# KogarashiNetwork/dusk-plonk

Hardware: AMD Instinct MI355X
Metric: PLONK prover constraints/sec (BLS12-381) at n=2^16 and 2^20, 1/2/4/8 GPUs (higher is better)
Workload: dtype u32-limb Montgomery Fr/Fp (integer)

## Files before the change

### dusk-plonk_amd/csrc/debug.hip

```cpp
#include <hip/hip_runtime.h>

#include <algorithm>
#include <vector>

#include "g1r.hpp"
#include "internal.hpp"
#include "prover.hpp"

namespace plk {
namespace {

template <class C>
__global__ void k_field_op(int op, const Fe<C>* __restrict__ a, const Fe<C>* __restrict__ b,
                           Fe<C>* __restrict__ out, uint64_t n) {
  const uint64_t i = (uint64_t)blockIdx.x * blockDim.x + threadIdx.x;
  if (i >= n) return;
  const Fe<C> x = a[i], y = b[i];
  Fe<C> r;
  switch (op) {
    case 0: r = fe_mul(x, y); break;
    case 1: r = fe_add(x, y); break;
    case 2: r = fe_sub(x, y); break;
    case 3: r = fe_sqr(x); break;
    default: r = fe_inv(x); break;
// ... 531 lines not shown
    plk::DeviceGuard g(key->ctx->device);
    hipStream_t s = key->ctx->stream;
    plk::DevBuf din, dout;
    int st;
    if ((st = din.alloc(len * sizeof(plk::Fr))) || (st = dout.alloc(total * sizeof(plk::Fr))))
      return st;
    PLK_HIP_TRY(hipMemcpyAsync(din.ptr, coef, len * sizeof(plk::Fr), hipMemcpyHostToDevice, s));
    plk::NttBatch b;
    b.in_stride = 0;
    b.out_stride = n;
    b.pre = key->coset_s.as<plk::Fr>();
    b.pre_stride = n + 8;
    if ((st = plk::ntt_run_batch(key->dom, din.as<plk::Fr>(), dout.as<plk::Fr>(), len, 1, 1,
                                 nullptr, s, (uint32_t)key->qb, b)))
      return st;
    PLK_HIP_TRY(hipMemcpyAsync(out, dout.ptr, total * sizeof(plk::Fr), hipMemcpyDeviceToHost, s));
    PLK_HIP_TRY(plk::stream_wait(s));
    return PLK_OK;
  } catch (...) {
    return PLK_E_DEVICE;
  }
}

extern "C" int plk_debug_prover_stage(plk_ctx* ctx, int stage, const uint64_t* const* in,
                                      const size_t* in_len, size_t n_in, const plk_fr* scalars,
                                      size_t n_scalars, const uint64_t* params, size_t n_params,
                                      uint64_t* out, size_t out_cap) {
  try {
    if (!ctx || stage < 0 || stage >= plk::kStCount) return PLK_E_ARG;
    if ((n_in && (!in || !in_len)) || (n_scalars && !scalars) || (n_params && !params) ||
        (out_cap && !out) || n_in > 32)
      return PLK_E_ARG;
    for (size_t k = 0; k < n_in; ++k)
      if (in_len[k] > ((size_t)1 << 28) || (in_len[k] && !in[k])) return PLK_E_ARG;
    const plk::StageCall c{stage, in, in_len, n_in, scalars, n_scalars, params, n_params, out, out_cap};
    plk::DeviceGuard g(ctx->device);
    return plk::run_stage(ctx, c);
  } catch (...) {
    return PLK_E_DEVICE;
  }
}
```

### dusk-plonk_amd/csrc/prover.hip

```cpp
#include <hip/hip_runtime.h>

#include <algorithm>
#include <cstring>
#include <memory>
#include <mutex>
#include <vector>

#include "ffr.hpp"
#include "internal.hpp"
#include "msm_common.hpp"
#include "prover.hpp"
#include "transcript.hpp"

using namespace plk;

namespace {

Fr fr_u64(uint64_t v) {
  Fr x = fe_zero<FrCfg>();
  x.v[0] = (uint32_t)v;
  x.v[1] = (uint32_t)(v >> 32);
  return fe_to_mont(x);
}
Fr fr_from(const plk_fr& a) {
// ... 267 lines not shown
  const size_t max_points = std::min<size_t>(std::min<size_t>(key->srs->n, key->n_trim), cap);
  std::vector<size_t> use(lens.size());
  for (size_t i = 0; i < lens.size(); ++i) use[i] = std::min(lens[i], max_points);
  int overall = PLK_OK;
  for (size_t base = 0; base < ptrs.size(); base += kMaxSlots) {
    const size_t m = std::min<size_t>(kMaxSlots, ptrs.size() - base);
    const int r = msm_run_batch(key->srs, ws, ptrs.data() + base, use.data() + base,
                                lens.data() + base, m, outs + base,
                                statuses ? statuses + base : nullptr, s, 0, 1, 0,
                                info ? info + base : nullptr);
    if (r != PLK_OK && r != PLK_E_DEGREE) return r;
    if (r != PLK_OK) overall = r;
  }
  return overall;
}

uint32_t lagrange_bucket_max(const plk_srs* s, size_t len) {
  const size_t dense = (size_t)s->windows * len >> (s->c - 1);
  return (uint32_t)std::max<size_t>(4 * kChunkMax, 4 * dense);
}

bool lagrange_commit_enabled() {
  const char* e = getenv("PLK_LAGRANGE_COMMIT");
  return !(e && e[0] == '0' && e[1] == 0);
}

int shard_commit(plk_prover* P, const std::vector<const Fr*>& ptrs,
                 const std::vector<size_t>& lens, plk_g1* outs, int* statuses, size_t cap) {
  plk_key* key = P->key;
  const size_t cnt = ptrs.size();
  const size_t max_points = std::min<size_t>(std::min<size_t>(key->srs->n, key->n_trim), cap);
  const bool buckets = P->shard_buckets;
  plk_srs* srs = buckets ? key->srs : P->shard;
  const uint64_t lo = buckets ? 0 : P->shard_lo, hi = buckets ? key->srs->n : lo + P->shard->n;
  const bool last = buckets || P->rank == P->world - 1;
  const uint32_t part = buckets ? (uint32_t)P->rank : 0, parts = buckets ? (uint32_t)P->world : 1;
  std::vector<const Fr*> lp(cnt);
  std::vector<size_t> luse(cnt), lchk(cnt);
  int local = PLK_OK;
  if (last && hi < max_points) local = PLK_E_ARG;
  for (size_t i = 0; i < cnt; ++i) {
    const size_t use = std::min(lens[i], max_points);
    luse[i] = use > lo ? (size_t)(std::min<uint64_t>(use, hi) - lo) : 0;
    lchk[i] = luse[i];
    lp[i] = ptrs[i] + lo;
    if (last && lens[i] > use) {
// ... 101 lines not shown
  qa.vk = fe_sqr(ch.var_sep);
  qa.vk2 = fe_sqr(qa.vk);
  qa.edwards_d = edwards_d();
  qa.has_fixed = has_fixed ? 1 : 0;
  qa.has_var = has_var ? 1 : 0;
  for (int j = 0; j < blocks; ++j) qa.vh_inv[j] = vh_inv[j];
  auto em1 = [](const Fr& x) { return fe_to_rx_domain(x); };
  auto em2 = [](const Fr& x) { return fe_to_rx_domain(fe_to_rx_domain(x)); };
  const Fr one = fe_one<FrCfg>(), two = fe_dbl(one);
  for (int mb = 0; mb < blocks; ++mb) qa.rx_bg[mb] = em2(fe_mul(ch.beta, s_m[mb]));
  qa.rx_beta = em2(ch.beta);
  qa.rx_gamma = em1(ch.gamma);
  qa.rx_one_w = em1(one);
  qa.rx_two_w = em1(two);
  qa.rx_three_w = em1(fe_add(two, one));
  qa.rx_kappa = em1(qa.kappa);
  qa.rx_kappa2 = em1(qa.kappa2);
  qa.rx_kappa3 = em1(qa.kappa3);
  qa.rx_alpha2 = em1(alpha2);
  for (int j = 0; j < blocks; ++j) qa.rx_vh[j] = em2(vh_inv[j]);
  qa.rx_32 = fr_u64(32);
  qa.rx_inv32 = fe_inv(qa.rx_32);
}
}

namespace plk {
namespace {
__global__ void k_sigma_values(const uint32_t* __restrict__ codes, const Fr* __restrict__ el,
                               uint64_t n, Fr k1, Fr k2, Fr k3, Fr* __restrict__ out) {
  const uint64_t i = (uint64_t)blockIdx.x * blockDim.x + threadIdx.x;
  if (i >= 4 * n) return;
  const uint32_t code = codes[i];
  const uint32_t g = code >> 2, col = code & 3;
  Fr v = el[g];
  if (col == 1) v = fe_mul(v, k1);
  if (col == 2) v = fe_mul(v, k2);
  if (col == 3) v = fe_mul(v, k3);
  out[i] = v;
}
}
}

extern "C" {

namespace {
std::mutex g_pool_mu;
// ... 336 lines not shown
    {
      const Fr gq = key->dom->g, one = fe_one<FrCfg>();
      Fr w8n;
      fr_root_of_unity(k + 3, w8n);
      const uint64_t rowc = n + 8;
      TRY(key->coset_s.alloc(QB * rowc * sizeof(Fr)));
      TRY(key->coset_w.alloc(QB * rowc * sizeof(Fr)));
      TRY(key->coset_pi.alloc(QB * rowc * sizeof(Fr)));
      TRY(key->icoset_q.alloc(QB * n * sizeof(Fr)));
      const Fr c32 = fr_u64(32);
      Fr sm = gq;
      for (int mb = 0; mb < QB; ++mb) {
        key->s_m[mb] = sm;
        TRY(ntt_power_table(key->coset_s.as<Fr>() + mb * rowc, sm, one, rowc, true, s));
        TRY(ntt_power_table(key->coset_w.as<Fr>() + mb * rowc, sm, c32, rowc, true, s));
        TRY(ntt_power_table(key->coset_pi.as<Fr>() + mb * rowc, sm, fe_inv(c32), rowc, true, s));
        TRY(ntt_power_table(key->icoset_q.as<Fr>() + mb * n, fe_inv(sm), key->dom->n_inv, n, true,
                            s));
        sm = fe_mul(sm, w8n);
      }
      Fr cm[kQBlocksMax];
      for (int mb = 0; mb < QB; ++mb) {
        cm[mb] = fe_pow_u64(key->s_m[mb], n);
        key->vh_inv[mb] = fe_inv(fe_sub(cm[mb], one));
      }
      for (int mb = 0; mb < QB; ++mb) {
        Fr poly[kQBlocksMax + 1];
        int deg = 0;
        poly[0] = one;
        Fr den = one;
        for (int j = 0; j < QB; ++j) {
          if (j == mb) continue;
          poly[deg + 1] = fe_zero<FrCfg>();
          for (int l = deg + 1; l >= 1; --l)
            poly[l] = fe_sub(poly[l - 1], fe_mul(poly[l], cm[j]));
          poly[0] = fe_neg(fe_mul(poly[0], cm[j]));
          ++deg;
          den = fe_mul(den, fe_sub(cm[mb], cm[j]));
        }
        const Fr dinv = fe_inv(den);
        for (int l = 0; l < QB; ++l) key->comb.m[l * QB + mb] = fe_to_rx_domain(fe_mul(poly[l], dinv));
      }
    }
    auto coset_fwd = [&](const Fr* in, Fr* out, uint64_t len, const DevBuf& table) {
      NttBatch b;
      b.in_stride = 0;
      b.out_stride = n;
      b.pre = table.as<Fr>();
      b.pre_stride = n + 8;
      return ntt_run_batch(key->dom, in, out, len, 1, 1, nullptr, s, QB, b);
    };
    TRY(key->selq.alloc(SEL_COUNTQ * nq * sizeof(Fr)));
    const int sel_src[SEL_COUNTQ] = {QM, QL, QR, QO, Q4, QC, QARITH, QRANGE, QLOGIC, QFIXED, QVAR};
    const bool sel_used[SEL_COUNTQ] = {true, true, true, true, true, true, true, key->has_range,
                                       key->has_logic, key->has_fixed, key->has_var};
    for (int j = 0; j < SEL_COUNTQ; ++j)
      if (sel_used[j])
        TRY(coset_fwd(qc + sel_src[j] * n, key->selq.as<Fr>() + j * nq, n, key->coset_s));
    TRY(key->sigmaq.alloc(4 * nq * sizeof(Fr)));
    for (int c = 0; c < 4; ++c)
      TRY(coset_fwd(sc + c * n, key->sigmaq.as<Fr>() + c * nq, n, key->coset_s));
    TRY(key->l1q.alloc(nq * sizeof(Fr)));
    {
      DevBuf tmp;
      TRY(tmp.alloc(n * sizeof(Fr)));
      TRY(pk_fill(tmp.as<Fr>(), key->dom->n_inv, n, s));
      TRY(coset_fwd(tmp.as<Fr>(), key->l1q.as<Fr>(), n, key->coset_s));
      PLK_HIP_TRY(stream_wait(s));
    }
    std::vector<uint32_t> idx(4 * n, 0);
    for (uint64_t i = 0; i < m; ++i)
      for (int c = 0; c < 4; ++c) {
        idx[c * n + i] = cs->gates[i].w[c];
        key->max_wire = std::max(key->max_wire, cs->gates[i].w[c]);
      }
    key->struct_hash = cs->struct_hash;
    TRY(key->wire_idx.alloc(4 * n * 4));
    PLK_HIP_TRY(hipMemcpyAsync(key->wire_idx.ptr, idx.data(), 4 * n * 4, hipMemcpyHostToDevice, s));
    PLK_HIP_TRY(stream_wait(s));
    *out = key.release();
    return PLK_OK;
  } catch (const std::bad_alloc&) {
    return PLK_E_OOM;
  } catch (...) {
    return PLK_E_DEVICE;
  }
}

int plk_key_destroy(plk_key* key) {
  if (!key) return PLK_E_ARG;
  DeviceGuard g(key->ctx->device);
  (void)stream_wait(key->ctx->stream);
  delete key;
  return PLK_OK;
}

int plk_key_info(const plk_key* key, uint64_t* n, uint64_t* m, plk_g1* commitments) {
  if (!key) return PLK_E_ARG;
  if (n) *n = key->n;
  if (m) *m = key->m;
  if (commitments) std::memcpy(commitments, key->comms, sizeof key->comms);
  return PLK_OK;
}

int plk_prover_create(plk_key* key, plk_prover** out) {
  try {
    if (!key || !out) return PLK_E_ARG;
    *out = nullptr;
    DeviceGuard guard(key->ctx->device);
    std::unique_ptr<plk_prover> p(new plk_prover());
    p->key = key;
    p->ws = msm_workspace_new();
    if (!p->ws->tail_forced) p->ws->tail_quad = lane_tail_policy(key->n);
    p->ws->shared_chip = true;
    PLK_HIP_TRY(hipStreamCreateWithFlags(&p->stream, hipStreamNonBlocking));
    p->own_stream = true;
    *out = p.release();
    return PLK_OK;
  } catch (const std::bad_alloc&) {
    return PLK_E_OOM;
  }
}

int plk_prover_destroy(plk_prover* p) {
// ... 126 lines not shown
    for (uint64_t i = 0; i < m; ++i)
      if (cs->gates[i].code & kPiBit) pis.emplace_back(i, gate_unpack(cs, i).pi);
    for (auto& p : pis) tr.append_scalar("pi", p.second);
    if (pi_count) *pi_count = pis.size();
    if (public_inputs)
      for (size_t i = 0; i < pis.size() && i < pi_cap; ++i) public_inputs[i] = fr_to(pis[i].second);

    {
      const size_t bytes = cs->witness.size() * sizeof(Fr);
      TRY(P->pin_witness.alloc(bytes));
      const size_t chunk = 8u << 20;
      const char* src = reinterpret_cast<const char*>(cs->witness.data());
      char* pin = P->pin_witness.as<char>();
      char* dst = P->witness.as<char>();
      for (size_t off = 0; off < bytes; off += chunk) {
        const size_t len = std::min(chunk, bytes - off);
        std::memcpy(pin + off, src + off, len);
        PLK_HIP_TRY(hipMemcpyAsync(dst + off, pin + off, len, hipMemcpyHostToDevice, s));
      }
    }
    Fr* wl = P->wires_lag.as<Fr>();
    Fr* wc = P->wires_coef.as<Fr>();
    TRY(pk_gather_wires(P->witness.as<Fr>(), key->wire_idx.as<uint32_t>(), m, n, wl, S, s));
    {
      NttBatch b;
      b.in_stride = S;
      b.out_stride = S;
      TRY(ntt_run_batch(key->dom, wl, wc, n, -1, 0, nsc, s, 4, b));
    }
    BlindBatch bb{};
    bb.npoly = 4;
    for (int c = 0; c < 4; ++c) {
      bb.poly[c] = wc + c * S;
      bb.lag[c] = wl + c * S;
      bb.b[c].count = 2;
      bb.b[c].r[0] = rng.fr();
      bb.b[c].r[1] = rng.fr();
    }
    TRY(pk_blind_batch(bb, n, s));
    plk_g1 wcom[4];
    {
      bool coef[4] = {true, true, true, true};
      for (int c = 0; c < 4; ++c) P->commit_basis[c] = 0, P->commit_entries[c] = 0;
      if (key->lag && !P->shard && !P->shard_buckets) {
        const Fr* ptrs[4] = {wl, wl + S, wl + 2 * S, wl + 3 * S};
        const size_t lens[4] = {n + 2, n + 2, n + 2, n + 2};
        MsmSlotInfo info[4];
        TRY(msm_run_batch(key->lag, *P->ws, ptrs, lens, lens, 4, wcom, nullptr, s, 0, 1,
                          lagrange_bucket_max(key->lag, n + 2), info));
        for (int c = 0; c < 4; ++c) {
          coef[c] = info[c].hot;
// ... 64 lines not shown
        pd.c[i] = fe_mul(pis[i].second, key->dom->n_inv);
      }
      TRY(pk_pi_coef(pd, key->dom->tw_inv.as<Fr>(), n, P->pi_coef.as<Fr>(), s));
    } else if (!pis.empty() && !pi_sparse) {
      PLK_HIP_TRY(hipMemsetAsync(pil, 0, n * sizeof(Fr), s));
      for (size_t i = 0; i < pis.size(); ++i) {
        P->pin_small.as<Fr>()[i] = pis[i].second;
        PLK_HIP_TRY(hipMemcpyAsync(pil + pis[i].first, P->pin_small.as<Fr>() + i, sizeof(Fr),
                                   hipMemcpyHostToDevice, s));
      }
    }
    Fr* ev = P->evq.as<Fr>();
    auto coset_fwd = [&](const Fr* in, Fr* out, uint64_t len, const DevBuf& table) {
      NttBatch b;
      b.in_stride = 0;
      b.out_stride = n;
      b.pre = table.as<Fr>();
      b.pre_stride = n + 8;
      return ntt_run_batch(key->dom, in, out, len, 1, 1, nsc, s, QB, b);
    };
    if (!pis.empty() && !pi_direct && !pi_sparse)
      TRY(ntt_run(key->dom, pil, P->pi_coef.as<Fr>(), n, -1, 0, nsc, s, 1));
    TRY(coset_fwd(zc, ev + 0 * nq, n + 3, key->coset_s));
    {
      NttBatch b;
      b.group = QB;
      b.in_stride = 0;
      b.in_group_stride = S;
      b.out_stride = n;
      b.pre = key->coset_w.as<Fr>();
      b.pre_stride = n + 8;
      TRY(ntt_run_batch(key->dom, wc, ev + nq, n + 2, 1, 1, nsc, s, 4 * QB, b));
    }
    if (pi_sparse) {
      PiSparse ps{};
      ps.count = (uint32_t)pis.size();
      for (size_t i = 0; i < pis.size(); ++i) {
        ps.idx[i] = (uint32_t)pis[i].first;
        ps.v[i] = pis[i].second;
      }
      TRY(pk_pi_sparse(ps, key->l1q.as<Fr>(), key->k, nq, ev + 5 * nq, s));
    } else if (!pis.empty()) {
      TRY(coset_fwd(P->pi_coef.as<Fr>(), ev + 5 * nq, n, key->coset_pi));
    }
    const Fr alpha2 = fe_sqr(alpha);
    QuotientArgs qa{};
    qa.z = ev;
    qa.a = ev + nq;
    qa.b = ev + 2 * nq;
    qa.c = ev + 3 * nq;
    qa.d = ev + 4 * nq;
    qa.pi = pis.empty() ? nullptr : ev + 5 * nq;
    qa.l1 = key->l1q.as<Fr>();
    qa.sel = key->selq.as<Fr>();
    qa.sigma = key->sigmaq.as<Fr>();
    qa.elements = key->dom->tw_fwd.as<Fr>();
// ... 252 lines not shown
```

### dusk-plonk_amd/csrc/prover.hpp

```cpp
#pragma once
#include <map>
#include <string>
#include <vector>

#include "internal.hpp"

namespace plk {

struct BlindArgs {
  Fr r[4];
  uint32_t count;
};
constexpr int kPiDirect = 16;
struct PiDirect {
  uint64_t idx[kPiDirect];
  Fr c[kPiDirect];
  uint32_t count;
};
struct BlindBatch {
  Fr* poly[4];
  Fr* lag[4];
  BlindArgs b[4];
  uint32_t npoly;
};

enum { SEL_QM = 0, SEL_QL, SEL_QR, SEL_QO, SEL_Q4, SEL_QC, SEL_QARITH, SEL_QRANGE, SEL_QLOGIC,
       SEL_QFIXED, SEL_QVAR, SEL_COUNTQ };

constexpr int kQBlocks = 5, kQBlocksSmall = 6, kQBlocksMax = 6;
inline int q_blocks(uint64_t n) { return n >= 16 ? kQBlocks : kQBlocksSmall; }
constexpr int kPiSparse = 4;
struct PiSparse {
  uint32_t count;
  uint32_t idx[kPiSparse];
  Fr v[kPiSparse];
};

struct QuotientArgs {
  const Fr *a, *b, *c, *d, *z, *pi, *l1, *sel, *sigma, *elements;
  Fr* out;
  uint64_t nq;
  uint32_t log_blk;
  Fr g, alpha, alpha2, beta, gamma, k1, k2, k3;
  Fr range_sep, kappa, kappa2, kappa3;
  Fr logic_sep, lk, lk2, lk3, lk4;
  Fr fixed_sep, fk, fk2, fk3;
  Fr var_sep, vk, vk2;
  Fr edwards_d;
  int has_range, has_logic, has_fixed, has_var;
  Fr vh_inv[kQBlocksMax];
  Fr rx_bg[kQBlocksMax], rx_beta, rx_gamma;
  Fr rx_one_w, rx_two_w, rx_three_w;
  Fr rx_kappa, rx_kappa2, rx_kappa3;
// ... 65 lines not shown
  return id;
}

PLK_HD Fr widget_var_base(const Fr& x1, const Fr& x3, const Fr& y1, const Fr& y3, const Fr& x2,
                          const Fr& y2, const Fr& x1y2, const Fr& k, const Fr& k2, const Fr& d) {
  const Fr xy_consistency = fe_sub(fe_mul(x1, y2), x1y2);
  const Fr y1x2 = fe_mul(y1, x2);
  const Fr y1y2 = fe_mul(y1, y2);
  const Fr x1x2 = fe_mul(x1, x2);
  const Fr dprod = fe_mul(fe_mul(d, x1y2), y1x2);
  const Fr x3c = fe_sub(fe_add(x1y2, y1x2), fe_add(x3, fe_mul(x3, dprod)));
  const Fr y3c = fe_sub(fe_add(y1y2, x1x2), fe_sub(y3, fe_mul(y3, dprod)));
  return fe_add(fe_add(xy_consistency, fe_mul(x3c, k)), fe_mul(y3c, k2));
}

int pk_gather_wires(const Fr* witness, const uint32_t* idx, uint64_t m, uint64_t n, Fr* out,
                    uint64_t stride, hipStream_t s);
int pk_blind(Fr* poly, uint64_t n, const BlindArgs& b, hipStream_t s);
int pk_blind_batch(const BlindBatch& bb, uint64_t n, hipStream_t s);
int pk_pi_coef(const PiDirect& pd, const Fr* tw_inv, uint64_t n, Fr* out, hipStream_t s);
int pk_pi_sparse(const PiSparse& ps, const Fr* l1, uint32_t log_n, uint64_t nq, Fr* out,
                 hipStream_t s);
int pk_fill(Fr* out, const Fr& v, uint64_t n, hipStream_t s);
int pk_perm_numden(const Fr* wires, uint64_t wire_stride, const Fr* sigmas, const Fr* elements,
                   uint64_t n, const Fr& beta, const Fr& gamma, const Fr& k1, const Fr& k2, const Fr& k3,
                   Fr* num, Fr* den, hipStream_t s);
int pk_mul3(const Fr* a, const Fr* b, const Fr& c, Fr* out, uint64_t n, hipStream_t s);
uint64_t pk_scan_tmp_elems(uint64_t n);
int pk_scan(const Fr* in, Fr* out, uint64_t n, bool mul, bool suffix, bool exclusive, Fr* tmp,
            hipStream_t s);
int pk_quotient(const QuotientArgs& q, hipStream_t s);
struct CombineMat {
  Fr m[kQBlocksMax * kQBlocksMax];
};
int pk_coset_combine(const Fr* in, uint64_t n, int blocks, const CombineMat& mat, Fr* out,
                     hipStream_t s);
int pk_scale_copy(const Fr* in, const Fr& c, Fr* out, uint64_t n, hipStream_t s);
uint32_t pk_eval_max_blocks(uint64_t max_len);
int pk_eval(const EvalBatch& e, uint32_t count, uint64_t max_len, Fr* partial, Fr* d_out,
            hipStream_t s);
int pk_lincomb(const LinComb& lc, Fr* out, uint64_t len_out, hipStream_t s);
int pk_scale_powers(const Fr* c, uint64_t len, const Fr& x, uint64_t shift, Fr* y, hipStream_t s);
int pk_ruffini(const Fr* c, uint64_t len, const Fr& z, Fr* q, Fr* tmp, Fr* scan_tmp,
               hipStream_t s);

struct Gate {
// ... 26 lines not shown

struct plk_key {
  plk_ctx* ctx = nullptr;
  plk_srs* srs = nullptr;
  std::string label;
  uint64_t m = 0, n = 0, n_trim = 0;
  uint32_t k = 0;
  plk_domain* dom = nullptr;
  plk_srs* lag = nullptr;
  int qb = 0;
  bool has_range = false, has_logic = false, has_fixed = false, has_var = false;
  plk::DevBuf q_coef;
  plk::DevBuf selq;
  plk::DevBuf sigma_coef;
  plk::DevBuf sigma_lag;
  plk::DevBuf sigmaq;
  plk::DevBuf l1q;
  plk::DevBuf coset_s, coset_w, coset_pi;
  plk::DevBuf icoset_q;
  plk::Fr s_m[plk::kQBlocksMax];
  plk::CombineMat comb;
  plk::DevBuf wire_idx;
  plk::Fr vh_inv[plk::kQBlocksMax];
  plk_g1 comms[15];
  uint64_t struct_hash = 0;
  uint32_t max_wire = 0;
  std::mutex def_mu;
  std::unique_ptr<plk_prover> def_prover;
  ~plk_key();
};

struct plk_prover {
  plk_key* key = nullptr;
  hipStream_t stream = nullptr;
  bool own_stream = false;
  plk::MsmWorkspace* ws = nullptr;
  plk_srs* shard = nullptr;
  uint64_t shard_lo = 0;
  bool shard_buckets = false;
  int rank = 0, world = 1;
  plk_allgather_fn allgather = nullptr;
  void* allgather_user = nullptr;
  plk::PinnedBuf pin_witness, pin_small;
  plk::PinnedBuf eval_out;
  void* eval_dev = nullptr;
  int commit_basis[4] = {0, 0, 0, 0};
// ... 6 lines not shown
```

### dusk-plonk_amd/csrc/prover_kernels.hip

```cpp
#include <hip/hip_runtime.h>

#include "ffr.hpp"
#include "internal.hpp"
#include "prover.hpp"

namespace plk {

namespace {

__device__ __forceinline__ Fr ldf(const Fr* p) {
  const uint4* q = reinterpret_cast<const uint4*>(p);
  uint4 a = q[0], b = q[1];
  Fr r;
  r.v[0] = a.x; r.v[1] = a.y; r.v[2] = a.z; r.v[3] = a.w;
  r.v[4] = b.x; r.v[5] = b.y; r.v[6] = b.z; r.v[7] = b.w;
  return r;
}

__device__ __forceinline__ void stf(Fr* p, const Fr& v) {
  uint4* q = reinterpret_cast<uint4*>(p);
  q[0] = make_uint4(v.v[0], v.v[1], v.v[2], v.v[3]);
  q[1] = make_uint4(v.v[4], v.v[5], v.v[6], v.v[7]);
}

// ... 46 lines not shown
    acc = rx_add(acc, rx_mul(rx_unpack(pd.c[k]), ldr(&tw_inv[(pd.idx[k] * j) & (n - 1)])));
  stf(&out[j], rx_pack_canonical(acc));
}

__global__ void __launch_bounds__(256) k_pi_sparse(PiSparse ps, const Fr* __restrict__ l1,
                                                   uint32_t log_n, uint64_t nq,
                                                   Fr* __restrict__ out) {
  const uint64_t i = (uint64_t)blockIdx.x * blockDim.x + threadIdx.x;
  if (i >= nq) return;
  const uint64_t mask = (1ull << log_n) - 1, base = i & ~mask, u = i & mask;
  RFr acc = rx_mul(ldr(&l1[base + ((u - ps.idx[0]) & mask)]), rx_unpack(ps.v[0]));
  for (uint32_t k = 1; k < ps.count; ++k)
    acc = rx_add(acc, rx_mul(ldr(&l1[base + ((u - ps.idx[k]) & mask)]), rx_unpack(ps.v[k])));
  stf(&out[i], rx_pack_canonical(acc));
}

__global__ void k_blind_batch(BlindBatch bb, uint64_t n) {
  const uint32_t p = threadIdx.x >> 2, i = threadIdx.x & 3;
  if (p >= bb.npoly || i >= bb.b[p].count) return;
  Fr* poly = bb.poly[p];
  stf(&poly[i], fe_sub(ldf(&poly[i]), bb.b[p].r[i]));
  stf(&poly[n + i], bb.b[p].r[i]);
  if (bb.lag[p]) stf(&bb.lag[p][n + i], bb.b[p].r[i]);
}

__global__ void k_fill(Fr* __restrict__ out, Fr v, uint64_t n) {
  const uint64_t i = (uint64_t)blockIdx.x * blockDim.x + threadIdx.x;
  if (i < n) stf(&out[i], v);
}

__global__ void k_perm_numden(const Fr* __restrict__ wires, uint64_t ws, const Fr* __restrict__ sigmas,
                              const Fr* __restrict__ elements, uint64_t n, Fr beta_rx, Fr gamma,
                              Fr k1_rx, Fr k2_rx, Fr k3_rx, Fr fix, Fr* __restrict__ num,
                              Fr* __restrict__ den) {
  const uint64_t i = (uint64_t)blockIdx.x * blockDim.x + threadIdx.x;
  if (i >= n) return;
  const RFr be = rx_unpack(beta_rx), g = rx_unpack(gamma);
  const RFr bx = rx_mul(be, ldr(&elements[i]));
  auto tn = [&](int c, const RFr& bxk) { return add3_u(ldr(&wires[c * ws + i]), g, bxk); };
  auto td = [&](int c) { return add3_u(ldr(&wires[c * ws + i]), g, rx_mul(be, ldr(&sigmas[c * n + i]))); };
  RFr nu = rx_norm(tn(0, bx)), de = rx_norm(td(0));
  nu = rx_mul(nu, tn(1, rx_mul(rx_unpack(k1_rx), bx)));
  de = rx_mul(de, td(1));
  nu = rx_mul(nu, tn(2, rx_mul(rx_unpack(k2_rx), bx)));
  de = rx_mul(de, td(2));
  nu = rx_mul(nu, tn(3, rx_mul(rx_unpack(k3_rx), bx)));
// ... 486 lines not shown

int pk_pi_coef(const PiDirect& pd, const Fr* tw_inv, uint64_t n, Fr* out, hipStream_t s) {
  if (pd.count > (uint32_t)kPiDirect || (n & (n - 1))) return PLK_E_ARG;
  hipLaunchKernelGGL(k_pi_coef, dim3(blocks_for(n, 256)), dim3(256), 0, s, pd, tw_inv, n, out);
  PLK_HIP_TRY(hipGetLastError());
  return PLK_OK;
}

int pk_pi_sparse(const PiSparse& ps, const Fr* l1, uint32_t log_n, uint64_t nq, Fr* out,
                 hipStream_t s) {
  if (ps.count == 0 || ps.count > (uint32_t)kPiSparse) return PLK_E_ARG;
  hipLaunchKernelGGL(k_pi_sparse, dim3(blocks_for(nq, 256)), dim3(256), 0, s, ps, l1, log_n, nq,
                     out);
  PLK_HIP_TRY(hipGetLastError());
  return PLK_OK;
}

int pk_blind_batch(const BlindBatch& bb, uint64_t n, hipStream_t s) {
  hipLaunchKernelGGL(k_blind_batch, dim3(1), dim3(64), 0, s, bb, n);
  PLK_HIP_TRY(hipGetLastError());
  return PLK_OK;
}

int pk_fill(Fr* out, const Fr& v, uint64_t n, hipStream_t s) {
  hipLaunchKernelGGL(k_fill, dim3(blocks_for(n, 256)), dim3(256), 0, s, out, v, n);
  PLK_HIP_TRY(hipGetLastError());
  return PLK_OK;
}

int pk_perm_numden(const Fr* wires, uint64_t wire_stride, const Fr* sigmas, const Fr* elements,
                   uint64_t n, const Fr& beta, const Fr& gamma, const Fr& k1, const Fr& k2, const Fr& k3,
                   Fr* num, Fr* den, hipStream_t s) {
  Fr fix = fe_zero<FrCfg>();
  fix.v[0] = 1;
  for (int b = 0; b < 4 * RxShape<FrCfg>::B * RxShape<FrCfg>::L - 3 * 256; ++b) fix = fe_dbl(fix);
  hipLaunchKernelGGL(k_perm_numden, dim3(blocks_for(n, 256)), dim3(256), 0, s, wires, wire_stride,
                     sigmas, elements, n, fe_to_rx_domain(beta), gamma, fe_to_rx_domain(k1),
                     fe_to_rx_domain(k2), fe_to_rx_domain(k3), fix, num, den);
  PLK_HIP_TRY(hipGetLastError());
  return PLK_OK;
}

int pk_mul3(const Fr* a, const Fr* b, const Fr& c, Fr* out, uint64_t n, hipStream_t s) {
  hipLaunchKernelGGL(k_mul3, dim3(blocks_for(n, 256)), dim3(256), 0, s, a, b, c, out, n);
  PLK_HIP_TRY(hipGetLastError());
  return PLK_OK;
// ... 137 lines not shown
```

### dusk-plonk_amd/plonk.py

```python
from __future__ import annotations

import ctypes as C
import os
from pathlib import Path

import numpy as np

_PKG = Path(__file__).resolve().parent
_LIB_PATH = Path(os.environ["PLK_LIB"]) if os.environ.get("PLK_LIB") else _PKG / "libplk.so"

PLK_OK, PLK_E_DEGREE, PLK_E_ARG, PLK_E_DEVICE, PLK_E_OOM, PLK_E_NODEV = range(6)

ABI_SYMBOLS = (
    "plk_abi_version", "plk_status_str", "plk_build_info", "plk_device_count", "plk_ctx_create",
    "plk_ctx_destroy", "plk_ctx_stream", "plk_ctx_synchronize", "plk_domain_get",
    "plk_domain_info", "plk_domain_elements", "plk_domain_vanishing_over_coset", "plk_ntt",
    "plk_ntt_dev", "plk_ntt_batch_dev", "plk_srs_setup", "plk_srs_load", "plk_srs_destroy",
    "plk_srs_len", "plk_srs_points", "plk_msm", "plk_commit", "plk_commit_dev",
    "plk_srs_last_msm_stats", "plk_debug_field_op", "plk_debug_rx_op", "plk_debug_g1r_op",
    "plk_debug_block_eval", "plk_debug_ntt_lazy_op", "plk_debug_prover_stage",
    "plk_commit_batch_dev",
    "plk_commit_batch_dev_part",
    "plk_srs_setup_range", "plk_g1_sum", "plk_msm_sharded", "plk_srs_msm_stats_reset",
    "plk_srs_cum_msm_stats", "plk_ntt_stream", "plk_aggregate_witness",
    "plk_aggregate_witness_dev",
    "plk_composer_create", "plk_composer_destroy", "plk_composer_size",
    "plk_composer_append_witness", "plk_composer_witness_value", "plk_composer_set_witness",
    "plk_composer_append_public", "plk_composer_append_gate", "plk_composer_append_custom_gate",
    "plk_composer_gate_eval", "plk_composer_assert_equal", "plk_composer_assert_equal_constant",
    "plk_composer_component_boolean", "plk_composer_component_range",
    "plk_composer_synthetic_chain",
    "plk_composer_public_inputs", "plk_composer_export", "plk_key_compile", "plk_key_destroy",
    "plk_key_info",
    "plk_prove", "plk_prover_create", "plk_prover_destroy", "plk_prover_stream",
    "plk_prover_prove", "plk_prover_msm_stats", "plk_prover_shard", "plk_prover_shard_buckets",
    "plk_proof_encode", "plk_proof_decode",
    "plk_msm_points", "plk_msm_points_ranges", "plk_verifier_create", "plk_verifier_destroy",
    "plk_verifier_challenges", "plk_verifier_fold", "plk_verifier_last_fold_stats",
    "plk_verifier_set_replay", "plk_verifier_challenges_batch", "plk_verifier_last_replay_ms",
    "plk_debug_fold_weights",
    "plk_srs_lagrange", "plk_prover_commit_info",
    "plk_opening_key_setup", "plk_opening_key_load", "plk_opening_key_points",
    "plk_opening_key_destroy", "plk_pairing_check", "plk_pairing_check_batch",
    "plk_opening_key_last_pairing_ms", "plk_debug_pairing", "plk_verifier_pairs",
    "plk_verifier_verify", "plk_verifier_verify_each", "plk_verifier_last_each_stats",
)


class PlonkError(RuntimeError):
    def __init__(self, status: int, what: str = ""):
        self.status = status
        msg = _lib().plk_status_str(status).decode() if _LIB is not None else str(status)
        super().__init__(f"{what}: {msg} (status {status})" if what else msg)


_LIB = None


def _lib():
    global _LIB
    if _LIB is None:
        if not _LIB_PATH.exists():
            raise ImportError(f"{_LIB_PATH} not built — run __graft_entry__.build() first")
        try:
# ... 625 lines not shown
```

### dusk-plonk_amd/prover.py

```python
from __future__ import annotations

import ctypes as C

import numpy as np

from .plonk import (PLK_OK, PlonkError, PlonkParams, _check, _lib, _ptr)

R_MOD = 0x73EDA753299D7D483339D80809A1D80553BDA402FFFE5BFEFFFFFFFF00000001
_R = 1 << 256


class PlkFr(C.Structure):
    _fields_ = [("l", C.c_uint64 * 4)]


class PlkG1(C.Structure):
    _fields_ = [("x", C.c_uint64 * 6), ("y", C.c_uint64 * 6), ("infinity", C.c_uint64)]


_SEL = ["q_m", "q_l", "q_r", "q_o", "q_4", "q_c", "q_arith", "q_range", "q_logic",
        "q_fixed_group_add", "q_variable_group_add"]


class PlkConstraint(C.Structure):
# ... 638 lines not shown
        except Exception:
            pass
        self._h = None


class Prover:
    def __init__(self, key_handle, n, m, label, pp):
        self._key, self.n, self.m, self.label, self.pp = key_handle, n, m, label, pp

    def create_proof(self, seed: int, circuit):
        cs = Plonk()
        circuit.synthesize(cs)
        return self.prove_composer(cs, seed)

    def prove_composer(self, cs: Plonk, seed: int):
        proof = PlkProof()
        pis = (PlkFr * 4096)()
        cnt = C.c_size_t()
        st = _bind().plk_prove(self._key, cs._h, seed, C.byref(proof), pis, 4096, C.byref(cnt))
        if st != PLK_OK:
            raise PlonkError(st, "create_proof")
        return Proof(proof), [fr_int(pis[i]) for i in range(cnt.value)]

    def lane(self) -> "ProverLane":
        return ProverLane(self)

    def __del__(self):
        try:
            for ln in list(getattr(self, "_lanes", [])):
                ln.close()
            if self._key:
                _bind().plk_key_destroy(self._key)
        except Exception:
            pass


class ProverLane:

    def __init__(self, prover: Prover):
        self.prover = prover
        self._h = C.c_void_p()
        _check(_bind().plk_prover_create(prover._key, C.byref(self._h)), "plk_prover_create")
        if not hasattr(prover, "_lanes"):
            prover._lanes = []
        prover._lanes.append(self)
        self._shard_keep = None
# ... 95 lines not shown
```

### include/plk.h

```cpp
#ifndef PLK_H
#define PLK_H

#include <stddef.h>
#include <stdint.h>

#ifdef __cplusplus
extern "C" {
#endif

#define PLK_ABI_VERSION 2

typedef struct { uint64_t l[4]; } plk_fr;
typedef struct { uint64_t x[6]; uint64_t y[6]; uint64_t infinity; } plk_g1;

typedef enum {
  PLK_OK = 0,
  PLK_E_DEGREE = 1,
  PLK_E_ARG = 2,
  PLK_E_DEVICE = 3,
  PLK_E_OOM = 4,
  PLK_E_NODEV = 5,
  PLK_E_UNSUPPORTED = 6
} plk_status;

// ... 89 lines not shown
int plk_composer_destroy(plk_composer* c);
int plk_composer_size(const plk_composer* c, size_t* gates, size_t* witnesses);
int plk_composer_append_witness(plk_composer* c, const plk_fr* value, uint32_t* wire);
int plk_composer_witness_value(const plk_composer* c, uint32_t wire, plk_fr* value);
int plk_composer_set_witness(plk_composer* c, uint32_t wire, const plk_fr* value);
int plk_composer_append_public(plk_composer* c, const plk_fr* value, uint32_t* wire);
int plk_composer_append_gate(plk_composer* c, const plk_constraint* s);
int plk_composer_append_custom_gate(plk_composer* c, const plk_constraint* s);
int plk_composer_gate_eval(plk_composer* c, const plk_constraint* s, uint32_t* out_wire);
int plk_composer_assert_equal(plk_composer* c, uint32_t a, uint32_t b);
int plk_composer_assert_equal_constant(plk_composer* c, uint32_t a, const plk_fr* constant,
                                       const plk_fr* public_input );
int plk_composer_component_boolean(plk_composer* c, uint32_t a);
int plk_composer_component_range(plk_composer* c, uint32_t a, size_t num_bits);
int plk_composer_synthetic_chain(plk_composer* c, size_t gates, uint64_t seed);
int plk_composer_public_inputs(const plk_composer* c, plk_fr* values, uint64_t* indexes,
                               size_t cap, size_t* count);
int plk_composer_export(const plk_composer* c, plk_constraint* gates, size_t cap,
                        plk_fr* witness, size_t wcap, size_t* m, size_t* nw);

int plk_key_compile(plk_srs* srs, const plk_composer* circuit, const char* label, plk_key** out);
int plk_key_destroy(plk_key* key);
int plk_key_info(const plk_key* key, uint64_t* n, uint64_t* m, plk_g1* commitments);
int plk_prove(plk_key* key, const plk_composer* circuit, uint64_t seed, plk_proof* proof,
              plk_fr* public_inputs, size_t pi_cap, size_t* pi_count);

typedef struct plk_prover plk_prover;
int plk_prover_create(plk_key* key, plk_prover** out);
int plk_prover_destroy(plk_prover* p);
int plk_prover_stream(plk_prover* p, void** stream_out);
int plk_prover_prove(plk_prover* p, const plk_composer* circuit, uint64_t seed, plk_proof* proof,
                     plk_fr* public_inputs, size_t pi_cap, size_t* pi_count);
int plk_prover_msm_stats(plk_prover* p, int reset, double* accumulate_ms, uint64_t* launches,
                         uint64_t* point_adds, uint64_t* points);
int plk_prover_commit_info(const plk_prover* p, int basis[4], uint64_t entries[4]);

typedef int (*plk_allgather_fn)(void* user, const void* send, size_t bytes, void* recv);
int plk_prover_shard(plk_prover* p, plk_srs* slice, uint64_t slice_start, int rank, int world,
                     plk_allgather_fn allgather, void* user);
int plk_prover_shard_buckets(plk_prover* p, int rank, int world, plk_allgather_fn allgather,
                             void* user);

typedef struct plk_verifier plk_verifier;
typedef struct { plk_g1 c, w; } plk_kzg_pair;

int plk_verifier_create(const char* label, uint64_t n, uint64_t m, const plk_g1 commitments[15],
// ... 30 lines not shown
int plk_verifier_pairs(plk_ctx* ctx, plk_verifier* v, const plk_proof* proofs,
                       const plk_fr* public_inputs, size_t count, plk_kzg_pair* out);
int plk_verifier_verify(plk_ctx* ctx, plk_verifier* v, const plk_opening_key* key,
                        const plk_proof* proofs, const plk_fr* public_inputs, size_t count,
                        const plk_fr* weights, int* ok);
int plk_verifier_verify_each(plk_ctx* ctx, plk_verifier* v, plk_opening_key* key,
                             const plk_proof* proofs, const plk_fr* public_inputs, size_t count,
                             uint8_t* ok);
int plk_verifier_last_each_stats(const plk_verifier* v, float* pairs_ms, float* pairing_ms);

#define PLK_PROOF_SCALE_BYTES (11 * 97 + 16 * 32)
int plk_proof_encode(const plk_proof* proof, uint8_t* out, size_t cap, size_t* len);
int plk_proof_decode(const uint8_t* in, size_t len, plk_proof* proof);

int plk_debug_field_op(plk_ctx* ctx, int field, int op, const uint64_t* a, const uint64_t* b,
                       uint64_t* out, size_t n);
int plk_debug_rx_op(plk_ctx* ctx, int field, int op, const uint32_t* a, const uint32_t* b,
                    const uint32_t* c, const uint32_t* d, uint32_t* out, size_t n);
int plk_debug_ntt_lazy_op(plk_ctx* ctx, int op, const uint32_t* in, uint32_t* out, size_t n);
int plk_debug_g1r_op(plk_ctx* ctx, int op, const uint32_t* p, const uint32_t* q,
                     const uint32_t* flags, uint32_t* out, size_t n);
int plk_debug_block_eval(plk_key* key, const uint64_t* coef, size_t len, uint64_t* out,
                         size_t out_cap, int* blocks_out);
int plk_debug_prover_stage(plk_ctx* ctx, int stage, const uint64_t* const* in, const size_t* in_len,
                           size_t n_in, const plk_fr* scalars, size_t n_scalars,
                           const uint64_t* params, size_t n_params, uint64_t* out, size_t out_cap);
int plk_debug_fold_weights(plk_ctx* ctx, const uint8_t entropy[32], const plk_fr* u, size_t count,
                           plk_fr* out);
int plk_debug_pairing(plk_ctx* ctx, const plk_g1* p, const plk_g2* q, size_t n, uint64_t* out);

#ifdef __cplusplus
}
#endif
#endif
```

Before: 36.82 million.

## Skip NTTs for zero or sparse wire columns using closed-form blinder coset evaluation

At key compile time, each wire column is classified as all-zero-wire or sparse (at most four gates use a non-zero wire index). At prove time, if witness[0] is zero, such columns skip the batched inverse NTT: they get a memset or a direct sparse coefficient computation. They also skip the forward coset NTT, replaced by a single kernel that evaluates the blinder polynomial plus a few Lagrange terms in closed form. This cuts NTT work in the wire-commit and quotient stages for circuits with unused wire columns. In exchange it adds more batched NTT launches split around skipped columns, new debug/query APIs, and an environment switch to disable it.

```diff
diff --git a/dusk-plonk_amd/csrc/debug.hip b/dusk-plonk_amd/csrc/debug.hip
--- a/dusk-plonk_amd/csrc/debug.hip
+++ b/dusk-plonk_amd/csrc/debug.hip
@@ -577,6 +577,71 @@
   }
 }
 
+extern "C" int plk_debug_blinder_coset(plk_key* key, const plk_fr* b, const uint32_t* gates,
+                                       const plk_fr* values, size_t count, uint64_t* closed,
+                                       uint64_t* transformed, size_t cap) {
+  using plk::Fr;
+  using plk::last_hip_error;
+  try {
+    if (!key || !b || count > (size_t)plk::kWireSparse || (count && (!gates || !values)))
+      return PLK_E_ARG;
+    const uint64_t n = key->n, S = n + 8, total = (uint64_t)key->qb * n;
+    if (cap < total) return PLK_E_ARG;
+    Fr val[plk::kWireSparse];
+    for (size_t k = 0; k < count; ++k) {
+      if (gates[k] >= n) return PLK_E_ARG;
+      val[k] = plk::fr_from_abi(values[k]);
+    }
+    plk::DeviceGuard g(key->ctx->device);
+    hipStream_t s = key->ctx->stream;
+    plk::DevBuf lag, coef, out;
+    int st;
+    if ((st = lag.alloc(n * sizeof(Fr))) || (st = coef.alloc(S * sizeof(Fr))) ||
+        (st = out.alloc(total * sizeof(Fr))))
+      return st;
+    const Fr b0 = plk::fr_from_abi(b[0]), b1 = plk::fr_from_abi(b[1]);
+    if (closed) {
+      plk::BlinderCoset bc{};
+      plk::blinder_coset_column(bc, key->s_m, key->vh, key->qb, b0, b1, gates, val, (uint32_t)count,
+                                out.as<Fr>());
+      if ((st = plk::pk_blinder_coset(bc, key->dom->tw_fwd.as<Fr>(), key->l1q.as<Fr>(), key->k,
+                                      key->qb, s)))
+        return st;
+      PLK_HIP_TRY(hipMemcpyAsync(closed, out.ptr, total * sizeof(Fr), hipMemcpyDeviceToHost, s));
+      PLK_HIP_TRY(plk::stream_wait(s));
+    }
+    if (transformed) {
+      PLK_HIP_TRY(hipMemsetAsync(lag.ptr, 0, n * sizeof(Fr), s));
+      for (size_t k = 0; k < count; ++k)
+        PLK_HIP_TRY(hipMemcpyAsync(lag.as<Fr>() + gates[k], &val[k], sizeof(Fr),
+                                   hipMemcpyHostToDevice, s));
+      PLK_HIP_TRY(hipMemsetAsync(coef.ptr, 0, S * sizeof(Fr), s));
+      if ((st = plk::ntt_run(key->dom, lag.as<Fr>(), coef.as<Fr>(), n, -1, 0, nullptr, s, 1)))
+        return st;
+      plk::BlindBatch bb{};
+      bb.npoly = 1;
+      bb.poly[0] = coef.as<Fr>();
+      bb.b[0].count = 2;
+      bb.b[0].r[0] = b0;
+      bb.b[0].r[1] = b1;
+      if ((st = plk::pk_blind_batch(bb, n, s))) return st;
+      plk::NttBatch nb;
+      nb.in_stride = 0;
+      nb.out_stride = n;
+      nb.pre = key->coset_w.as<Fr>();
+      nb.pre_stride = n + 8;
+      if ((st = plk::ntt_run_batch(key->dom, coef.as<Fr>(), out.as<Fr>(), n + 2, 1, 1, nullptr, s,
+                                   (uint32_t)key->qb, nb)))
+        return st;
+      PLK_HIP_TRY(hipMemcpyAsync(transformed, out.ptr, total * sizeof(Fr), hipMemcpyDeviceToHost, s));
+      PLK_HIP_TRY(plk::stream_wait(s));
+    }
+    return PLK_OK;
+  } catch (...) {
+    return PLK_E_DEVICE;
+  }
+}
+
 extern "C" int plk_debug_prover_stage(plk_ctx* ctx, int stage, const uint64_t* const* in,
                                       const size_t* in_len, size_t n_in, const plk_fr* scalars,
                                       size_t n_scalars, const uint64_t* params, size_t n_params,
diff --git a/dusk-plonk_amd/csrc/prover.hip b/dusk-plonk_amd/csrc/prover.hip
--- a/dusk-plonk_amd/csrc/prover.hip
+++ b/dusk-plonk_amd/csrc/prover.hip
@@ -313,6 +313,11 @@
 
 bool lagrange_commit_enabled() {
   const char* e = getenv("PLK_LAGRANGE_COMMIT");
+  return !(e && e[0] == '0' && e[1] == 0);
+}
+
+bool zero_column_enabled() {
+  const char* e = getenv("PLK_ZERO_COLUMN");
   return !(e && e[0] == '0' && e[1] == 0);
 }
 
@@ -460,6 +465,24 @@
   qa.rx_32 = fr_u64(32);
   qa.rx_inv32 = fe_inv(qa.rx_32);
 }
+
+void blinder_coset_column(BlinderCoset& bc, const Fr* s_m, const Fr* vh, int blocks, const Fr& b0,
+                          const Fr& b1, const uint32_t* gate, const Fr* value, uint32_t count,
+                          Fr* out) {
+  const uint32_t col = bc.ncol++;
+  const Fr c32 = fr_u64(32);
+  bc.out[col] = out;
+  for (int mb = 0; mb < blocks; ++mb) {
+    const Fr v = fe_mul(c32, vh[mb]);
+    bc.a[col][mb] = fe_mul(b0, v);
+    bc.b[col][mb] = fe_mul(fe_mul(b1, s_m[mb]), v);
+  }
+  bc.count[col] = count;
+  for (uint32_t k = 0; k < count && k < (uint32_t)kWireSparse; ++k) {
+    bc.idx[col][k] = gate[k];
+    bc.v[col][k] = fe_mul(c32, value[k]);
+  }
+}
 }
 
 namespace plk {
@@ -842,7 +865,8 @@
       Fr cm[kQBlocksMax];
       for (int mb = 0; mb < QB; ++mb) {
         cm[mb] = fe_pow_u64(key->s_m[mb], n);
-        key->vh_inv[mb] = fe_inv(fe_sub(cm[mb], one));
+        key->vh[mb] = fe_sub(cm[mb], one);
+        key->vh_inv[mb] = fe_inv(key->vh[mb]);
       }
       for (int mb = 0; mb < QB; ++mb) {
         Fr poly[kQBlocksMax + 1];
@@ -889,11 +913,24 @@
       PLK_HIP_TRY(stream_wait(s));
     }
     std::vector<uint32_t> idx(4 * n, 0);
+    for (int c = 0; c < 4; ++c) key->sparse_cnt[c] = 0;
     for (uint64_t i = 0; i < m; ++i)
       for (int c = 0; c < 4; ++c) {
-        idx[c * n + i] = cs->gates[i].w[c];
-        key->max_wire = std::max(key->max_wire, cs->gates[i].w[c]);
-      }
+        const uint32_t w = cs->gates[i].w[c];
+        idx[c * n + i] = w;
+        key->max_wire = std::max(key->max_wire, w);
+        int& cnt = key->sparse_cnt[c];
+        if (w == 0 || cnt < 0) continue;
+        if (cnt == kWireSparse) {
+          cnt = -1;
+          continue;
+        }
+        key->sparse_gate[c][cnt] = (uint32_t)i;
+        key->sparse_wire[c][cnt] = w;
+        ++cnt;
+      }
+    for (int c = 0; c < 4; ++c) key->zero_col[c] = key->sparse_cnt[c] == 0;
+    key->zero_fast = zero_column_enabled();
     key->struct_hash = cs->struct_hash;
     TRY(key->wire_idx.alloc(4 * n * 4));
     PLK_HIP_TRY(hipMemcpyAsync(key->wire_idx.ptr, idx.data(), 4 * n * 4, hipMemcpyHostToDevice, s));
@@ -920,6 +957,18 @@
   if (n) *n = key->n;
   if (m) *m = key->m;
   if (commitments) std::memcpy(commitments, key->comms, sizeof key->comms);
+  return PLK_OK;
+}
+
+int plk_key_zero_columns(const plk_key* key, int out[4]) {
+  if (!key || !out) return PLK_E_ARG;
+  for (int c = 0; c < 4; ++c) out[c] = key->zero_col[c] ? 1 : 0;
+  return PLK_OK;
+}
+
+int plk_key_sparse_columns(const plk_key* key, int count[4]) {
+  if (!key || !count) return PLK_E_ARG;
+  for (int c = 0; c < 4; ++c) count[c] = key->sparse_cnt[c];
   return PLK_OK;
 }
 
@@ -1092,11 +1141,34 @@
     Fr* wl = P->wires_lag.as<Fr>();
     Fr* wc = P->wires_coef.as<Fr>();
     TRY(pk_gather_wires(P->witness.as<Fr>(), key->wire_idx.as<uint32_t>(), m, n, wl, S, s));
+    bool skip[4];
     {
+      const bool zero_w = key->zero_fast && !cs->witness.empty() && fe_is_zero(cs->witness[0]);
+      for (int c = 0; c < 4; ++c) skip[c] = zero_w && key->sparse_cnt[c] >= 0;
+    }
+    for (int c0 = 0; c0 < 4;) {
+      if (skip[c0]) {
+        if (key->sparse_cnt[c0] == 0) {
+          PLK_HIP_TRY(hipMemsetAsync(wc + c0 * S, 0, n * sizeof(Fr), s));
+        } else {
+          PiDirect pd{};
+          pd.count = (uint32_t)key->sparse_cnt[c0];
+          for (uint32_t k = 0; k < pd.count; ++k) {
+            pd.idx[k] = key->sparse_gate[c0][k];
+            pd.c[k] = fe_mul(cs->witness[key->sparse_wire[c0][k]], key->dom->n_inv);
+          }
+          TRY(pk_pi_coef(pd, key->dom->tw_inv.as<Fr>(), n, wc + c0 * S, s));
+        }
+        ++c0;
+        continue;
+      }
+      int c1 = c0 + 1;
+      while (c1 < 4 && !skip[c1]) ++c1;
       NttBatch b;
       b.in_stride = S;
       b.out_stride = S;
-      TRY(ntt_run_batch(key->dom, wl, wc, n, -1, 0, nsc, s, 4, b));
+      TRY(ntt_run_batch(key->dom, wl + c0 * S, wc + c0 * S, n, -1, 0, nsc, s, (uint32_t)(c1 - c0), b));
+      c0 = c1;
     }
     BlindBatch bb{};
     bb.npoly = 4;
@@ -1207,7 +1279,19 @@
     if (!pis.empty() && !pi_direct && !pi_sparse)
       TRY(ntt_run(key->dom, pil, P->pi_coef.as<Fr>(), n, -1, 0, nsc, s, 1));
     TRY(coset_fwd(zc, ev + 0 * nq, n + 3, key->coset_s));
-    {
+    BlinderCoset bc{};
+    for (int c0 = 0; c0 < 4;) {
+      if (skip[c0]) {
+        Fr val[kWireSparse];
+        for (int k = 0; k < key->sparse_cnt[c0]; ++k) val[k] = cs->witness[key->sparse_wire[c0][k]];
+        blinder_coset_column(bc, key->s_m, key->vh, QB, bb.b[c0].r[0], bb.b[c0].r[1],
+                             key->sparse_gate[c0], val, (uint32_t)key->sparse_cnt[c0],
+                             ev + (1 + c0) * nq);
+        ++c0;
+        continue;
+      }
+      int c1 = c0 + 1;
+      while (c1 < 4 && !skip[c1]) ++c1;
       NttBatch b;
       b.group = QB;
       b.in_stride = 0;
@@ -1215,8 +1299,11 @@
       b.out_stride = n;
       b.pre = key->coset_w.as<Fr>();
       b.pre_stride = n + 8;
-      TRY(ntt_run_batch(key->dom, wc, ev + nq, n + 2, 1, 1, nsc, s, 4 * QB, b));
-    }
+      TRY(ntt_run_batch(key->dom, wc + c0 * S, ev + (1 + c0) * nq, n + 2, 1, 1, nsc, s,
+                        (uint32_t)((c1 - c0) * QB), b));
+      c0 = c1;
+    }
+    TRY(pk_blinder_coset(bc, key->dom->tw_fwd.as<Fr>(), key->l1q.as<Fr>(), key->k, QB, s));
     if (pi_sparse) {
       PiSparse ps{};
       ps.count = (uint32_t)pis.size();
diff --git a/dusk-plonk_amd/csrc/prover.hpp b/dusk-plonk_amd/csrc/prover.hpp
--- a/dusk-plonk_amd/csrc/prover.hpp
+++ b/dusk-plonk_amd/csrc/prover.hpp
@@ -29,6 +29,16 @@
 
 constexpr int kQBlocks = 5, kQBlocksSmall = 6, kQBlocksMax = 6;
 inline int q_blocks(uint64_t n) { return n >= 16 ? kQBlocks : kQBlocksSmall; }
+constexpr int kWireSparse = 4;
+struct BlinderCoset {
+  Fr* out[4];
+  Fr a[4][kQBlocksMax];
+  Fr b[4][kQBlocksMax];
+  uint32_t count[4];
+  uint32_t idx[4][kWireSparse];
+  Fr v[4][kWireSparse];
+  uint32_t ncol;
+};
 constexpr int kPiSparse = 4;
 struct PiSparse {
   uint32_t count;
@@ -140,6 +150,11 @@
 int pk_pi_sparse(const PiSparse& ps, const Fr* l1, uint32_t log_n, uint64_t nq, Fr* out,
                  hipStream_t s);
 int pk_fill(Fr* out, const Fr& v, uint64_t n, hipStream_t s);
+void blinder_coset_column(BlinderCoset& bc, const Fr* s_m, const Fr* vh, int blocks, const Fr& b0,
+                          const Fr& b1, const uint32_t* gate, const Fr* value, uint32_t count,
+                          Fr* out);
+int pk_blinder_coset(const BlinderCoset& bc, const Fr* elements, const Fr* l1, uint32_t log_n,
+                     int blocks, hipStream_t s);
 int pk_perm_numden(const Fr* wires, uint64_t wire_stride, const Fr* sigmas, const Fr* elements,
                    uint64_t n, const Fr& beta, const Fr& gamma, const Fr& k1, const Fr& k2, const Fr& k3,
                    Fr* num, Fr* den, hipStream_t s);
@@ -212,6 +227,12 @@
   plk::CombineMat comb;
   plk::DevBuf wire_idx;
   plk::Fr vh_inv[plk::kQBlocksMax];
+  plk::Fr vh[plk::kQBlocksMax];
+  bool zero_col[4] = {false, false, false, false};
+  int sparse_cnt[4] = {-1, -1, -1, -1};
+  uint32_t sparse_gate[4][plk::kWireSparse] = {};
+  uint32_t sparse_wire[4][plk::kWireSparse] = {};
+  bool zero_fast = true;
   plk_g1 comms[15];
   uint64_t struct_hash = 0;
   uint32_t max_wire = 0;
diff --git a/dusk-plonk_amd/csrc/prover_kernels.hip b/dusk-plonk_amd/csrc/prover_kernels.hip
--- a/dusk-plonk_amd/csrc/prover_kernels.hip
+++ b/dusk-plonk_amd/csrc/prover_kernels.hip
@@ -92,6 +92,19 @@
   stf(&poly[i], fe_sub(ldf(&poly[i]), bb.b[p].r[i]));
   stf(&poly[n + i], bb.b[p].r[i]);
   if (bb.lag[p]) stf(&bb.lag[p][n + i], bb.b[p].r[i]);
+}
+
+__global__ void __launch_bounds__(256) k_blinder_coset(BlinderCoset bc, const Fr* __restrict__ elements,
+                                                       const Fr* __restrict__ l1, uint32_t log_n) {
+  const uint64_t n = 1ull << log_n, mask = n - 1;
+  const uint64_t u = (uint64_t)blockIdx.x * blockDim.x + threadIdx.x;
+  const uint32_t m = blockIdx.y, col = blockIdx.z;
+  if (u >= n) return;
+  const uint64_t base = (uint64_t)m * n;
+  Fr acc = fe_add(bc.a[col][m], fe_mul(bc.b[col][m], ldf(&elements[u])));
+  for (uint32_t k = 0; k < bc.count[col]; ++k)
+    acc = fe_add(acc, fe_mul(bc.v[col][k], ldf(&l1[base + ((u - bc.idx[col][k]) & mask)])));
+  stf(&bc.out[col][base + u], acc);
 }
 
 __global__ void k_fill(Fr* __restrict__ out, Fr v, uint64_t n) {
@@ -624,6 +637,19 @@
   return PLK_OK;
 }
 
+int pk_blinder_coset(const BlinderCoset& bc, const Fr* elements, const Fr* l1, uint32_t log_n,
+                     int blocks, hipStream_t s) {
+  if (bc.ncol == 0) return PLK_OK;
+  if (bc.ncol > 4 || blocks < 1 || blocks > kQBlocksMax || log_n > 27) return PLK_E_ARG;
+  for (uint32_t c = 0; c < bc.ncol; ++c)
+    if (bc.count[c] > (uint32_t)kWireSparse) return PLK_E_ARG;
+  const uint64_t n = 1ull << log_n;
+  hipLaunchKernelGGL(k_blinder_coset, dim3(blocks_for(n, 256), (unsigned)blocks, bc.ncol), dim3(256),
+                     0, s, bc, elements, l1, log_n);
+  PLK_HIP_TRY(hipGetLastError());
+  return PLK_OK;
+}
+
 int pk_fill(Fr* out, const Fr& v, uint64_t n, hipStream_t s) {
   hipLaunchKernelGGL(k_fill, dim3(blocks_for(n, 256)), dim3(256), 0, s, out, v, n);
   PLK_HIP_TRY(hipGetLastError());
diff --git a/dusk-plonk_amd/plonk.py b/dusk-plonk_amd/plonk.py
--- a/dusk-plonk_amd/plonk.py
+++ b/dusk-plonk_amd/plonk.py
@@ -40,6 +40,7 @@
     "plk_verifier_set_replay", "plk_verifier_challenges_batch", "plk_verifier_last_replay_ms",
     "plk_debug_fold_weights",
     "plk_srs_lagrange", "plk_prover_commit_info",
+    "plk_key_zero_columns", "plk_key_sparse_columns", "plk_debug_blinder_coset",
     "plk_opening_key_setup", "plk_opening_key_load", "plk_opening_key_points",
     "plk_opening_key_destroy", "plk_pairing_check", "plk_pairing_check_batch",
     "plk_opening_key_last_pairing_ms", "plk_debug_pairing", "plk_verifier_pairs",
diff --git a/dusk-plonk_amd/prover.py b/dusk-plonk_amd/prover.py
--- a/dusk-plonk_amd/prover.py
+++ b/dusk-plonk_amd/prover.py
@@ -684,6 +684,35 @@
             raise PlonkError(st, "create_proof")
         return Proof(proof), [fr_int(pis[i]) for i in range(cnt.value)]
 
+    def _columns(self, name):
+        f = getattr(_bind(), name)
+        f.restype, f.argtypes = C.c_int, [C.c_void_p, C.POINTER(C.c_int)]
+        out = (C.c_int * 4)()
+        _check(f(self._key, out), name)
+        return [int(v) for v in out]
+
+    def zero_columns(self):
+        return [bool(v) for v in self._columns("plk_key_zero_columns")]
+
+    def sparse_columns(self):
+        return self._columns("plk_key_sparse_columns")
+
+    def blinder_coset(self, b0, b1, gates=(), values=()):
+        f = _bind().plk_debug_blinder_coset
+        f.restype = C.c_int
+        f.argtypes = [C.c_void_p, C.c_void_p, C.c_void_p, C.c_void_p, C.c_size_t, C.c_void_p,
+                      C.c_void_p, C.c_size_t]
+        blocks = 5 if self.n >= 16 else 6
+        b = (PlkFr * 2)(_fr(b0), _fr(b1))
+        cnt = len(gates)
+        g = (C.c_uint32 * max(cnt, 1))(*gates)
+        v = (PlkFr * max(cnt, 1))(*[_fr(x) for x in values])
+        closed = np.zeros((blocks * self.n, 4), dtype=np.uint64)
+        transformed = np.zeros((blocks * self.n, 4), dtype=np.uint64)
+        _check(f(self._key, b, g, v, cnt, _ptr(closed), _ptr(transformed), blocks * self.n),
+               "plk_debug_blinder_coset")
+        return closed, transformed
+
     def lane(self) -> "ProverLane":
         return ProverLane(self)
 
diff --git a/include/plk.h b/include/plk.h
--- a/include/plk.h
+++ b/include/plk.h
@@ -135,6 +135,8 @@
 int plk_key_compile(plk_srs* srs, const plk_composer* circuit, const char* label, plk_key** out);
 int plk_key_destroy(plk_key* key);
 int plk_key_info(const plk_key* key, uint64_t* n, uint64_t* m, plk_g1* commitments);
+int plk_key_zero_columns(const plk_key* key, int out[4]);
+int plk_key_sparse_columns(const plk_key* key, int count[4]);
 int plk_prove(plk_key* key, const plk_composer* circuit, uint64_t seed, plk_proof* proof,
               plk_fr* public_inputs, size_t pi_cap, size_t* pi_count);
 
@@ -211,6 +213,9 @@
                      const uint32_t* flags, uint32_t* out, size_t n);
 int plk_debug_block_eval(plk_key* key, const uint64_t* coef, size_t len, uint64_t* out,
                          size_t out_cap, int* blocks_out);
+int plk_debug_blinder_coset(plk_key* key, const plk_fr* b, const uint32_t* gates,
+                            const plk_fr* values, size_t count, uint64_t* closed,
+                            uint64_t* transformed, size_t cap);
 int plk_debug_prover_stage(plk_ctx* ctx, int stage, const uint64_t* const* in, const size_t* in_len,
                            size_t n_in, const plk_fr* scalars, size_t n_scalars,
                            const uint64_t* params, size_t n_params, uint64_t* out, size_t out_cap);
```

After: 37.10 million, median of 4. No clear change (+0.8%).
